# roljon/Steered-Mixture-of-Experts

Measured on AMD Instinct MI355X. Metric: Mpixel-iters/s (SMoE fit: forward + analytic backward + TF1 Adam), 16x16 blocks / 4 kernels, higher is better.
Workload: dtype f32

## Files before the change

### steered_mixture_of_experts_amd/csrc/smoe_block.hip.h

```cpp
#ifndef SMOE_BLOCK_HIP_H
#define SMOE_BLOCK_HIP_H

#include <hip/hip_runtime.h>
#include <stdint.h>

#include <type_traits>

#include "smoe_device.h"
#include "smoe_ssim.hip.h"
#include "smoe_fq.hip.h"

namespace smoe {


__device__ __forceinline__ float fast_rcp(float x) { return __builtin_amdgcn_rcpf(x); }

__device__ __forceinline__ uint32_t hw_wave_slot() {
    return __builtin_amdgcn_s_getreg(4 | (0 << 6) | ((4 - 1) << 11));
}
__device__ __forceinline__ void rotate_priority(int it, uint32_t slot) {
    const uint32_t pr = ((uint32_t)it + slot) % 3u;
    if (pr == 0u) __builtin_amdgcn_s_setprio(0);
    else if (pr == 1u) __builtin_amdgcn_s_setprio(1);
    else __builtin_amdgcn_s_setprio(2);
// ... 118 lines not shown
    __device__ __forceinline__ float nu(int k, int c) const { return P[k * Lt::PK + Lt::O_NU + c]; }
    __device__ __forceinline__ float ga(int k, int l, int c) const { return P[k * Lt::PK + Lt::O_GA + l * C + c]; }
    __device__ __forceinline__ bool flag(int k) const { return P[Lt::LP_ACT + k] != 0.0f; }
    __device__ __forceinline__ bool frozen() const { return P[Lt::LP_FROZEN] != 0.0f; }
    __device__ __forceinline__ bool act(int k) const { return flag(k) && (pi(k) > 0.0f); }

    __device__ __forceinline__ void load(const float* __restrict__ lds_block) {
        const float4* src = reinterpret_cast<const float4*>(lds_block);
#pragma unroll
        for (int i = 0; i < Lt::LP_STRIDE / 4; ++i) {
            const float4 q = src[i];
            P[4 * i + 0] = q.x; P[4 * i + 1] = q.y; P[4 * i + 2] = q.z; P[4 * i + 3] = q.w;
        }
    }

    template <bool IC = false>
    __device__ __forceinline__ void derive(const KernelConsts& kc) {
#pragma unroll
        for (int k = 0; k < K; ++k) {
            float det = 1.0f;
#pragma unroll
            for (int l = 0; l < D; ++l) det *= A(k, l, l);
            const float nq = kc.use_det ? det * kc.inv_n_dis : 1.0f;
            coef[k] = act(k) ? nq * pi(k) : 0.0f;
#pragma unroll
            for (int l = 0; l < D; ++l)
#pragma unroll
                for (int m = 0; m <= l; ++m)
                    As[k][tri_index(l, m)] = (IC ? ((l == m) ? SMOE_SQ * SMOE_SQ : 2.0f * SMOE_SQ * SMOE_SQ) : SMOE_SQ) * A(k, l, m);
#pragma unroll
            for (int m = 0; m < D; ++m) {
                float c = 0.0f;
                if (!IC) {
#pragma unroll
                    for (int l = m; l < D; ++l) c = fmaf(mu(k, l), As[k][tri_index(l, m)], c);
                }
                cz[k][m] = c;
            }
            if (!kc.train_gammas) {
#pragma unroll
                for (int i = 0; i < D * C; ++i) P[k * Lt::PK + Lt::O_GA + i] = 0.0f;
            }
            if (kc.only_y_gamma) {
#pragma unroll
// ... 156 lines not shown
            float h = R.nu(k, c);
#pragma unroll
            for (int l = D - HL; l < D; ++l) h = fmaf(R.ga(k, l, c), xc[l], h);
            R.he[k][c] = h;
        }
    }
}

template <int D, int C, int K>
struct PixelOut {
    float wt[K];
    float q[C];
    float kq[C];
};

template <int D, int C, int K, bool TRAIN, int HL = 0, bool EXTG = false, bool IC = false, bool FLAGS = false, bool RAWLOSS = false>
__device__ __forceinline__ void pixel(const BlockRegs<D, C, K>& R, const KernelConsts& kc,
                                      const float (&x)[D], const float (&t)[C], float lw,
                                      float* __restrict__ acc, PixelOut<D, C, K>& o,
                                      const float* __restrict__ gext = nullptr,
                                      unsigned long long* __restrict__ flags = nullptr, bool fed = true,
                                      float* __restrict__ lraw = nullptr, unsigned long long fedm = ~0ull) {
    using Lt = Layout<D, C, K>;
    float z[K][D], g[K];
    float S = 0.0f;
#pragma unroll
    for (int k = 0; k < K; ++k) {
        float maha = 0.0f;
        if (IC) {
            maha = (HL > 0) ? R.hq[k] : 0.0f;
#pragma unroll
// ... 37 lines not shown
#pragma unroll
            for (int l = 0; l < D - HL; ++l) ee = fmaf(R.ga(k, l, c), x[l], ee);
            e[k][c] = ee;
            y[c] = (k == 0) ? o.wt[k] * ee : fmaf(o.wt[k], ee, y[c]);
        }
    }
    float Gc[C];
    float dot = 0.0f;
#pragma unroll
    for (int c = 0; c < C; ++c) {
        const float yc = __builtin_amdgcn_fmed3f(y[c], 0.0f, kc.nudged_max);
        o.kq[c] = floorf(fmaf(yc, kc.inv_scale, 0.5f));
        o.q[c] = o.kq[c] * kc.scale;
        const float diff = o.q[c] - t[c];
        const float ad = fabsf(diff) - kc.epsm;
        acc[Lt::S_SSE] = fmaf(diff, diff, acc[Lt::S_SSE]);
        const float cwl = kc.cw[c] * lw;
        if constexpr (RAWLOSS) lraw[c] = fmaf(ad, ad, lraw[c]);
        else if (!EXTG) acc[Lt::S_LOSS] = fmaf(cwl, ad * ad, acc[Lt::S_LOSS]);
        if (TRAIN) {
            const float c2 = cwl + cwl;
            const float gm = EXTG ? gext[c] : ad * __builtin_amdgcn_fmed3f(diff * 1.2676506e30f, -c2, c2);
            Gc[c] = (yc == y[c]) ? gm : 0.0f;
            dot = (c == 0) ? Gc[c] * y[c] : fmaf(Gc[c], y[c], dot);
        }
    }
    if (!TRAIN) return;
    dot = (S > 10e-12f) ? dot : 0.0f;
    float Gx[(D - HL > 0) ? D - HL : 1][C];
#pragma unroll
    for (int l = 0; l < D - HL; ++l)
// ... 62 lines not shown
            for (int c = 0; c < C; ++c) a[Lt::O_GA + l * C + c] = xc[l] * a[Lt::O_NU + c];
        }
    }
}

template <int D, int C, int K>
__device__ __forceinline__ void tie_diagonal(float* __restrict__ a) {
    using Lt = Layout<D, C, K>;
    float tr = 0.0f;
#pragma unroll
    for (int l = 0; l < D; ++l) tr += a[Lt::O_A + tri_index(l, l)];
#pragma unroll
    for (int l = 0; l < D; ++l) a[Lt::O_A + tri_index(l, l)] = tr;
}

template <int D, int C, int K, bool IC = false>
__device__ __forceinline__ void finish_partials(const BlockRegs<D, C, K>& R, const KernelConsts& kc,
                                                float* __restrict__ acc) {
    using Lt = Layout<D, C, K>;
#pragma unroll
    for (int k = 0; k < K; ++k) {
        float* a = acc + k * Lt::PK;
        const bool act = R.act(k);
        const float su = a[Lt::O_PI];
        if (IC) {
            float sur[D];
#pragma unroll
            for (int l = 0; l < D; ++l) sur[l] = a[Lt::O_MU + l];
#pragma unroll
            for (int l = 0; l < D; ++l) {
                float gm = 0.0f;
#pragma unroll
                for (int m = 0; m < D; ++m) gm = fmaf((l >= m) ? R.A(k, l, m) : R.A(k, m, l), sur[m], gm);
                a[Lt::O_MU + l] = gm;
// ... 11 lines not shown
        float suz[D];
#pragma unroll
        for (int m = 0; m < D; ++m) suz[m] = a[Lt::O_MU + m] * SMOE_INV_SQ;
#pragma unroll
        for (int l = 0; l < D; ++l) {
            float gm = 0.0f;
#pragma unroll
            for (int m = 0; m <= l; ++m) gm = fmaf(R.A(k, l, m), suz[m], gm);
            a[Lt::O_MU + l] = gm;
        }
#pragma unroll
        for (int l = 0; l < D; ++l) {
#pragma unroll
            for (int m = 0; m <= l; ++m) {
                float v = fmaf(R.mu(k, l), suz[m], -(a[Lt::O_A + tri_index(l, m)] * SMOE_INV_SQ));
                if (l == m && kc.use_det) v = fmaf(su, act ? fast_rcp(R.A(k, l, l)) : 0.0f, v);
                a[Lt::O_A + tri_index(l, m)] = v;
            }
        }
        a[Lt::O_PI] = su * (act ? fast_rcp(R.pi(k)) : 0.0f);
        if (kc.radial) tie_diagonal<D, C, K>(a);
    }
}

struct SlotDesc {
    float c_self, pub_scale;
    uint32_t T1, T2, T3, TR, P1, P2, P3, PR, FLAG, PIV;
};

template <int D, int C, int K, bool IC>
__device__ __forceinline__ SlotDesc build_slot_desc(int j, uint32_t tot_base, uint32_t img_base, uint32_t par_base,
                                                    bool patch_pis, bool use_det) {
    using Lt = Layout<D, C, K>;
    const uint32_t ZERO = par_base + 4u * Lt::LP_ZERO, ONE = par_base + 4u * Lt::LP_ONE;
    const int k = j / Lt::PK, o = j - k * Lt::PK;
// ... 97 lines not shown
    __host__ __device__ static constexpr int tgt_stride(int N) { return C * N + TGT_PAD; }
    __host__ __device__ static constexpr int lw_stride(int N) { return N + TGT_PAD; }
    
    __host__ __device__ static int off_coords() { return 0; }
    __host__ __device__ static int off_par(int N, int CR) { return round_up(CR * N, 4); }
    __host__ __device__ static int off_mv(int N, int CR) { return off_par(N, CR) + NB * Lt::LP_STRIDE; }
    static constexpr bool OWNER_POST = (G >= 64);
    static constexpr int DESC_DW = 12;
    static constexpr int DESC_STRIDE = OWNER_POST ? Lt::NPAR * DESC_DW : 0;
    static constexpr int TOT_STRIDE = round_up(Lt::NSLOT, 4);
    static_assert(!OWNER_POST || BPW * TOT_STRIDE <= CH * ROW, "the published totals must fit into the reduction scratch");
    __host__ __device__ static bool wants_owner_post(int N) { return OWNER_POST && N <= 8 * G; }
    __host__ __device__ static int off_scratch(int N, int CR) { return off_mv(N, CR) + NB * MV_STRIDE; }
    __host__ __device__ static int off_tgt(int N, int CR) { return off_scratch(N, CR) + WAVES * CH * ROW; }
    __host__ __device__ static int off_lw(int N, int CR) { return off_tgt(N, CR) + NB * tgt_stride(N); }
    __host__ __device__ static size_t bytes(int N, bool has_lw, int CR = D, bool hq = false) {
        return sizeof(float) * (size_t)off_ssim(N, has_lw, CR, hq);
    }
    static constexpr int QI_RNG = 40;
    static constexpr int QI_OUT = 12;
    static constexpr int QI_STRIDE = round_up(Lt::LP_STRIDE + QI_RNG + QI_OUT, 4);
    __host__ __device__ static int off_qimg(int N, bool has_lw, int CR) { return round_up(off_lw(N, CR) + (has_lw ? NB * lw_stride(N) : 0), 4); }
    __host__ __device__ static int off_ssim(int N, bool has_lw, int CR, bool hq = false) { return off_qimg(N, has_lw, CR) + (hq ? NB * QI_STRIDE : 0); }
    __host__ __device__ static int ssim_tabs(int bh, int bw, int bt = 0) { return (G == 16) ? 0 : round_up(11 * (bh + bw + bt), 4); }
    __host__ __device__ static int ssim_wave(int N) { return (G == 16) ? BPW * C * N : round_up(C * N + ((D == 3) ? 10 : 8) * N, 4); }
    __host__ __device__ static size_t bytes_ssim(int N, bool has_lw, int CR, int bh, int bw, bool hq = false, int bt = 0) {
        return sizeof(float) * (size_t)(off_ssim(N, has_lw, CR, hq) + ssim_tabs(bh, bw, bt) + WAVES * ssim_wave(N));
    }
};

template <int D, int C, int K, int G, int WAVES, int CR = D>
__device__ __forceinline__ void stage_inputs(const float* __restrict__ coords, const float* __restrict__ target,
// ... 322 lines not shown
        float4 r = row[0];
#pragma unroll
        for (int i = 1; i < G / 4; ++i) {
            const float4 q = row[i];
            if (MIN) { r.x = fminf(r.x, q.x); r.y = fminf(r.y, q.y); r.z = fminf(r.z, q.z); r.w = fminf(r.w, q.w); }
            else { r.x += q.x; r.y += q.y; r.z += q.z; r.w += q.w; }
        }
        s_out[sub] = MIN ? fminf(fminf(r.x, r.y), fminf(r.z, r.w)) : (r.x + r.y) + (r.z + r.w);
    }
    wave_lds_sync();
#pragma unroll
    for (int i = 0; i < 10; ++i) v[i] = s_out[i];
    wave_lds_sync();
}

template <int D, int C, int K, bool HAS_LW, int HL, bool IC = false>
__device__ __forceinline__ void pixel_loop_train(const BlockRegs<D, C, K>& R, const KernelConsts& kc,
                                                 const float* __restrict__ s_coords, const float* __restrict__ s_tgt,
                                                 const float* __restrict__ s_lw, int N, int G, int sub,
                                                 float* __restrict__ acc, bool sample = false) {
    const int pxl = (N + G - 1) / G;
    const int full = N / G;
    unsigned long long flags[K];
#pragma unroll
    for (int k = 0; k < K; ++k) flags[k] = 0ull;
    constexpr bool RAWL = !HAS_LW;
    const unsigned long long not_sampled = sample ? 0ull : ~0ull;
    float lraw[C];
#pragma unroll
    for (int c = 0; c < C; ++c) lraw[c] = 0.0f;
    auto step = [&](int i) {
        const int n = i * G + sub;
        float x[D], t[C];
#pragma unroll
        for (int l = 0; l < D; ++l) x[l] = (l < D - HL) ? s_coords[l * N + n] : 0.0f;
#pragma unroll
        for (int c = 0; c < C; ++c) t[c] = s_tgt[c * N + n];
        const float lw = HAS_LW ? s_lw[n] : 1.0f;
        PixelOut<D, C, K> o;
        const bool fed = !(HAS_LW && sample) || lw != 0.0f;
        unsigned long long fedm = ~0ull;
        if constexpr (HAS_LW) fedm = __ballot(lw != 0.0f) | not_sampled;
        pixel<D, C, K, true, HL, false, IC, true, RAWL>(R, kc, x, t, lw, acc, o, nullptr, flags, fed, lraw, fedm);
    };
    int i = 0;
    if (full > 0) { step(0); i = 1; }
    if constexpr (D == 2 && C == 3) {
        for (; i < full; ++i) step(i);
    } else {
        for (; i + 1 < full; i += 2) { step(i); step(i + 1); }
        if (i < full) step(i);
    }
    if (full < pxl) {
        const int n = full * G + sub;
        if (n < N) {
            float x[D], t[C];
#pragma unroll
            for (int l = 0; l < D; ++l) x[l] = (l < D - HL) ? s_coords[l * N + n] : 0.0f;
#pragma unroll
            for (int c = 0; c < C; ++c) t[c] = s_tgt[c * N + n];
            const float lw = HAS_LW ? s_lw[n] : 1.0f;
            PixelOut<D, C, K> o;
            pixel<D, C, K, true, HL, false, IC, false, RAWL>(R, kc, x, t, lw, acc, o, nullptr, nullptr, !(HAS_LW && sample) || lw != 0.0f, lraw);
        }
    }
    if constexpr (RAWL) {
#pragma unroll
        for (int c = 0; c < C; ++c) acc[Layout<D, C, K>::S_LOSS] = fmaf(kc.cw[c], lraw[c], acc[Layout<D, C, K>::S_LOSS]);
    }
    const int lane = threadIdx.x & 63;
#pragma unroll
    for (int k = 0; k < K; ++k) acc[Layout<D, C, K>::S_CNT + k] += ((flags[k] >> lane) & 1ull) ? 1.0f : 0.0f;
}

template <int D, int C, int K, int G, int HL, bool SSIM, bool QUANT>
constexpr int fit_min_waves() {
    return ((G == 64 || (G == 16 && SMOE_W2_G16) || (G == 32 && SMOE_W2_G32)) && HL >= 1 && !SSIM && !QUANT && Layout<D, C, K>::NSLOT >= ((G == 64) ? SMOE_W2_SLOTS : 90)
            && Layout<D, C, K>::NSLOT <= SMOE_W2_SLOTS_MAX) ? 2 : 1;
}

template <int D, int C, int K, int G, int WAVES, int HL, bool SSIM = false, bool QUANT = false, bool IC = false, bool PAIR = false>
__global__ void __launch_bounds__(WAVES * 64) __attribute__((amdgpu_waves_per_eu(fit_min_waves<D, C, K, G, HL, SSIM, QUANT>()))) fit_kernel(FitArgs a) {
    using Lt = Layout<D, C, K>;
    using T = Tile<D, C, K, G, WAVES>;
    static_assert(!PAIR || (G == 64 && WAVES == 2 && !SSIM && !QUANT), "PAIR: one block on the two wavefronts of a workgroup");
    extern __shared__ __attribute__((aligned(16))) float lds[];
    const int N = a.N;
    const int B = a.B;
    const int wave = threadIdx.x >> 6;
    const int lane = threadIdx.x & 63;
    const int grp = lane / G;
    const int sub = lane - grp * G;
    const int blk0 = blockIdx.x * (PAIR ? 1 : T::NB);
    const int lb = PAIR ? 0 : wave * T::BPW + grp;
// ... 1 lines not shown
    const int b_raw = blk0 + lb;
    const bool valid_b = b_raw < B;
    const int b = valid_b ? b_raw : B - 1;

    constexpr int CR = D - HL;
    float* s_coords = lds + T::off_coords();
    float* s_par = lds + T::off_par(N, CR) + lb * Lt::LP_STRIDE;
    float* s_mv = lds + T::off_mv(N, CR) + lb * T::MV_STRIDE;
    float* s_scratch = lds + T::off_scratch(N, CR) + wave * (T::CH * T::ROW);
    const bool owner_post = T::OWNER_POST && a.desc_off > 0;
    float* s_desc = lds + a.desc_off + lb * T::DESC_STRIDE;
    float* s_tot = s_scratch + grp * T::TOT_STRIDE;
    const float* s_tgt = lds + T::off_tgt(N, CR) + lb * T::tgt_stride(N);
    const float* s_lw = lds + T::off_lw(N, CR) + lb * T::lw_stride(N);
    const bool has_lw = a.loss_w != nullptr;

    SMOE_LDS_CHECK(T::off_ssim(N, has_lw, CR, QUANT) + (SSIM ? T::ssim_tabs(a.bh, a.bw, (D == 3) ? a.bt : 0) + WAVES * T::ssim_wave(N) : 0), 1u);
    if (owner_post) SMOE_LDS_CHECK(a.desc_off + T::NB * T::DESC_STRIDE, 2u);
    stage_inputs<D, C, K, G, WAVES, CR>(a.coords, a.target, a.loss_w, B, N, blk0, lds);
    float* s_q = lds + T::off_qimg(N, has_lw, CR) + lb * T::QI_STRIDE;
    float* s_rng = s_q + Lt::LP_STRIDE;
    float* s_out = s_rng + T::QI_RNG;
    float* s_ssim = lds + T::off_ssim(N, has_lw, CR, QUANT);
    const int bh = a.bh, bw = a.bw, bt = (D == 3) ? a.bt : 0;
    const float* s_Tr = s_ssim;
    const float* s_Tc = s_ssim + bh * 11;
    const float* s_Tt = s_Tc + bw * 11;
    float* s_X = s_ssim + T::ssim_tabs(bh, bw, bt) + wave * T::ssim_wave(N) + ((G == 16) ? grp * (C * N) : 0);
    float* s_Wa = s_X + C * N;
    float* s_Wb = s_Wa + 5 * N;
    float wj[11];
    if (SSIM) {
// ... 30 lines not shown
            int tensor, kern; long off;
            decode_slot<D, C, K>(j, b, tensor, off, kern);
            s_par[j] = pick(a.p, tensor)[off];
            s_mv[2 * j] = pick(a.m, tensor)[off];
            s_mv[2 * j + 1] = pick(a.v, tensor)[off];
            float r = (tensor == 0) ? a.lr_pis : ((tensor == 2 || tensor == 3) ? a.lr_steer : a.lr_expert);
            if (tensor == 0 && !a.train_pis) r = 0.0f;
            if (tensor == 1 && !a.train_musx) r = 0.0f;
            if (tensor == 4 && !a.kc.train_gammas) r = 0.0f;
            if (tensor == 4 && a.kc.only_y_gamma && (off % C) != 0) r = 0.0f;
            if (tensor == 3 && a.kc.radial) r = 0.0f;
            lr[s] = r;
            reg[s] = (tensor == 0) ? a.reg_pi : ((tensor == 2) ? (a.kc.radial ? a.reg_u * (float)D : a.reg_u) : 0.0f);
            const int qg = (tensor == 0) ? 3 : ((tensor == 1) ? 1 : ((tensor == 4) ? 4 : ((tensor == 5) ? 2 : 0)));
            meta[s] = tensor | (kern << 4);
            if constexpr (QUANT) {
                if (tensor == 1 && a.mus_grid != nullptr && a.kc.qmode >= 2) goff[s] = a.mus_grid[off];
                if ((tensor == 0 && a.kc.qpis) || (tensor != 0 && a.kc.qmode == 2)) {
                    qlo[s] = a.kc.q_nmin[qg]; qhi[s] = a.kc.q_nmax[qg]; qsc[s] = a.kc.q_scale[qg]; qiv[s] = a.kc.q_inv[qg];
                }
                if (a.kc.qmode == 3 && tensor != 0 && !(tensor == 1 && !a.kc.q_musx))
                    qt[s] = (tensor == 2) ? 0 : ((tensor == 3) ? 1 : ((tensor == 1) ? 2 : ((tensor == 5) ? 3 : 4)));
            } else {
                (void)qg;
            }
        } else if (j >= Lt::S_CNT && j < Lt::S_CNT + K) {
            const int k = j - Lt::S_CNT;
            s_par[Lt::LP_ACT + k] = ((a.active[b] >> k) & 1u) ? 1.0f : 0.0f;
        } else if (j == Lt::S_LOSS) {
            s_par[Lt::LP_FROZEN] = (a.diverged != nullptr && a.diverged[b] != 0u) ? 1.0f : 0.0f;
        }
    }
    const float loss0 = (a.loss0 != nullptr) ? a.loss0[b] : 0.0f;
    const bool has_loss0 = a.loss0 != nullptr;
    const bool has_reg = (a.reg_pi != 0.0f) || (a.reg_u != 0.0f);
    const bool has_quant = (a.kc.qmode != 0) || (a.kc.qpis != 0);
    float last_loss = no_pass_value(), last_sse = no_pass_value();
    __syncthreads();

    auto pick5 = [](const float (&v)[10], int base, int t) {
        return (t == 0) ? v[base] : ((t == 1) ? v[base + 1] : ((t == 2) ? v[base + 2] : ((t == 3) ? v[base + 3] : v[base + 4])));
    };
    auto refresh_quantised_image = [&]() {
        if constexpr (QUANT) {
            if (a.kc.qmode == 3) {
                constexpr float INF = __builtin_huge_valf();
                float ex[10];
#pragma unroll
                for (int i = 0; i < 10; ++i) ex[i] = INF;
                const FqRange rp = fq_fixed(a.kc, 3);
#pragma unroll
                for (int s = 0; s < T::SPL; ++s) {
                    const int j = T::slot_of(sub, s);
                    if (j < Lt::NPAR && qt[s] >= 0) {
                        const bool keep = fq_val(s_par[(meta[s] >> 4) * Lt::PK + Lt::O_PI], rp) > 0.0f;
                        const float x = s_par[j] - goff[s];
#pragma unroll
                        for (int t = 0; t < 5; ++t) {
                            const bool hit = keep && (qt[s] == t);
                            ex[t] = hit ? fminf(ex[t], x) : ex[t];
                            ex[5 + t] = hit ? fminf(ex[5 + t], -x) : ex[5 + t];
                        }
                    }
                }
                block_allreduce10<G, T::ROW, true>(ex, s_scratch, s_out, lane, grp, sub);
                {
                    const int t = min(sub, 4);
                    float lo = pick5(ex, 0, t), hi = -pick5(ex, 5, t);
                    if (lo == INF) { lo = 0.0f; hi = 0.0f; }
                    if (t == 1) { lo = fminf(lo, 0.0f); hi = fmaxf(hi, 0.0f); }
// ... 3 lines not shown
                        float* o = s_rng + t * 8;
                        o[0] = r.nmin; o[1] = r.nmax; o[2] = r.scale; o[3] = r.inv;
                        o[4] = r.back; o[5] = r.zero ? 1.0f : 0.0f; o[6] = lo; o[7] = hi;
                    }
                }
                wave_lds_sync();
            }
        }
        if constexpr (!QUANT) {
#pragma unroll
            for (int s = 0; s < T::SPL; ++s) {
                const int j = T::slot_of(sub, s);
                if (meta[s] >= 0 && (meta[s] & 15) == 0) {
                    const float x = s_par[j];
                    const float cl = fminf(fmaxf(x, a.kc.q_nmin[3]), a.kc.q_nmax[3]);
                    s_par[Lt::LP_QPI + (meta[s] >> 4)] = floorf((cl - a.kc.q_nmin[3]) * a.kc.q_inv[3] + 0.5f) * a.kc.q_scale[3] + a.kc.q_nmin[3];
                }
            }
            wave_lds_sync();
            return;
        }
        if constexpr (QUANT) {
#pragma unroll
        for (int s = 0; s < T::SPL; ++s) {
            const int j = T::slot_of(sub, s);
            if (j < Lt::NPAR) {
                const float x = s_par[j] - goff[s];
                float q = x;
                if (qsc[s] != 0.0f) {
                    const float cl = fminf(fmaxf(x, qlo[s]), qhi[s]);
                    q = floorf((cl - qlo[s]) * qiv[s] + 0.5f) * qsc[s] + qlo[s];
// ... 8 lines not shown
                    }
                }
                s_q[j] = q + goff[s];
            } else if (j >= Lt::S_CNT && j < Lt::S_CNT + K) {
                s_q[Lt::LP_ACT + (j - Lt::S_CNT)] = s_par[Lt::LP_ACT + (j - Lt::S_CNT)];
            } else if (j == Lt::S_LOSS) {
                s_q[Lt::LP_FROZEN] = s_par[Lt::LP_FROZEN];
            }
        }
        }
        wave_lds_sync();
    };
    if (has_quant) refresh_quantised_image();
    const float* s_img = (QUANT && has_quant) ? s_q : s_par;
    const bool patch_pis = !QUANT && (a.kc.qpis != 0);
    if (owner_post && !helper) {
        const uint32_t tot_off = (uint32_t)((s_tot - lds) * sizeof(float));
        const uint32_t img_off = (uint32_t)((s_img - lds) * sizeof(float));
        const uint32_t par_off = (uint32_t)((s_par - lds) * sizeof(float));
#pragma unroll
        for (int s = 0; s < T::SPL; ++s) {
            const int j = T::slot_of(sub, s);
            if (j < Lt::NPAR) {
                const SlotDesc d = build_slot_desc<D, C, K, IC>(j, tot_off, img_off, par_off, patch_pis, a.kc.use_det != 0);
                float4* o = reinterpret_cast<float4*>(s_desc + j * T::DESC_DW);
                o[0] = make_float4(d.c_self, d.pub_scale, __uint_as_float(d.T1), __uint_as_float(d.T2));
                o[1] = make_float4(__uint_as_float(d.T3), __uint_as_float(d.TR), __uint_as_float(d.P1), __uint_as_float(d.P2));
                o[2] = make_float4(__uint_as_float(d.P3), __uint_as_float(d.PR), __uint_as_float(d.FLAG), __uint_as_float(d.PIV));
            } else if (j == Lt::S_LOSS) {
                s_par[Lt::LP_ZERO] = 0.0f;
// ... 16 lines not shown
    for (int it = 0; it < a.n_iters; ++it) {
        if (a.prio_rotate) rotate_priority(it, hw_wave_slot());
        else if (phase_prio) __builtin_amdgcn_s_setprio(0);
        float acc[Lt::NSLOT];
#pragma unroll
        for (int j = 0; j < Lt::NSLOT; ++j) acc[j] = 0.0f;
        bool frozen;
        float reg_loss = 0.0f;
        {
            BlockRegs<D, C, K> R;
            R.load(s_img);
            if (patch_pis) {
#pragma unroll
                for (int k = 0; k < K; ++k) R.P[k * Lt::PK + Lt::O_PI] = R.P[Lt::LP_QPI + k];
            }
            R.template derive<IC>(kc);
            frozen = R.frozen();
            if (has_reg) {
                const float rp = kc.kcount_norm ? kc.pis_l1_raw / count_pis<D, C, K>(R.P) : reg_pi;
#pragma unroll
                for (int k = 0; k < K; ++k) {
                    if (R.act(k)) {
                        reg_loss += rp * R.pi(k);
#pragma unroll
                        for (int l = 0; l < D; ++l) reg_loss += reg_u * R.A(k, l, l);
                    }
                }
            }
            if (HL > 0) hoist_const<D, C, K, HL, IC>(R, xc);
#if SMOE_SGPR_CONSTS
            if constexpr (G == 64 && !SSIM && !QUANT && !IC && HL >= 1 && K * C >= 24) {
// ... 42 lines not shown
                    float x[D], t[C], gq[C];
#pragma unroll
                    for (int l = 0; l < D; ++l) x[l] = (l < D - HL) ? s_coords[l * N + n] : 0.0f;
#pragma unroll
                    for (int c = 0; c < C; ++c) { t[c] = s_tgt[c * N + n]; gq[c] = s_X[c * N + n]; }
                    PixelOut<D, C, K> o;
                    pixel<D, C, K, true, HL, true, IC, decltype(voted)::value>(R, kc, x, t, 1.0f, acc, o, gq, flags);
                };
                for (int i = 0; i < full; ++i) grad_step(i * G + sub, std::true_type{});
                for (int i = full; i < pxl; ++i)
                    if (i * G + sub < N) grad_step(i * G + sub, std::false_type{});
#pragma unroll
                for (int k = 0; k < K; ++k) acc[Lt::S_CNT + k] += ((flags[k] >> lane) & 1ull) ? 1.0f : 0.0f;
            } else {
                const int gl = PAIR ? 2 * G : G, sl = PAIR ? wave * G + sub : sub;
                if (has_lw) pixel_loop_train<D, C, K, true, HL, IC>(R, kc, s_coords, s_tgt, s_lw, N, gl, sl, acc, a.lw_is_sample != 0);
                else pixel_loop_train<D, C, K, false, HL, IC>(R, kc, s_coords, s_tgt, s_lw, N, gl, sl, acc);
            }
            if (HL > 0) complete_const<D, C, K, HL, IC>(R, xc, acc);
            SMOE_CLK(1);
        }
        if (phase_prio) __builtin_amdgcn_s_setprio(3);
        if (!owner_post) {
            BlockRegs<D, C, K> R2;
            R2.load(s_img);
            if (patch_pis) {
#pragma unroll
                for (int k = 0; k < K; ++k) R2.P[k * Lt::PK + Lt::O_PI] = R2.P[Lt::LP_QPI + k];
            }
            finish_partials<D, C, K, IC>(R2, kc, acc);
        }

        SMOE_CLK(2);
        float total[T::SPL];
        reduce_slots<D, C, K, G, WAVES, 0>(acc, s_scratch, lane, total);
        SMOE_CLK(3);

        if constexpr (PAIR) {
            float* s_x = lds + T::off_scratch(N, CR) + (T::CH * T::ROW);
            if (helper) {
                wave_lds_sync();
#pragma unroll
                for (int s = 0; s < T::SPL; ++s) {
                    const int j = T::slot_of(sub, s);
                    if (j < Lt::NSLOT) s_x[j] = total[s];
// ... 90 lines not shown
            if (kc.qmode == 3) {
                float rs[10], cn[10];
                bool bel[T::SPL], abv[T::SPL], tlo[T::SPL], thi[T::SPL];
#pragma unroll
                for (int i = 0; i < 10; ++i) { rs[i] = 0.0f; cn[i] = 0.0f; }
                const FqRange rp = fq_fixed(kc, 3);
#pragma unroll
                for (int s = 0; s < T::SPL; ++s) {
                    const int j = T::slot_of(sub, s);
                    bel[s] = abv[s] = tlo[s] = thi[s] = false;
                    if (j < Lt::NPAR && qt[s] >= 0) {
                        const float* o = s_rng + qt[s] * 8;
                        const bool unshifted = qt[s] == 0 && kc.radial;
                        const float x = s_par[j] - goff[s], v = unshifted ? x : x - o[4];
                        const bool zero = o[5] != 0.0f;
                        const bool keep = fq_val(s_par[(meta[s] >> 4) * Lt::PK + Lt::O_PI], rp) > 0.0f;
                        bel[s] = !zero && (v < o[0]);
                        abv[s] = !zero && (v > o[1]);
                        tlo[s] = keep && (x == o[6]);
                        thi[s] = keep && (x == o[7]);
#pragma unroll
                        for (int t = 0; t < 5; ++t) {
                            const bool hit = qt[s] == t;
                            rs[t] += (hit && (unshifted ? !abv[s] : bel[s])) ? gq[s] : 0.0f;
                            rs[5 + t] += (hit && abv[s]) ? gq[s] : 0.0f;
                            cn[t] += (hit && tlo[s]) ? 1.0f : 0.0f;
                            cn[5 + t] += (hit && thi[s]) ? 1.0f : 0.0f;
                        }
                    }
                }
                block_allreduce10<G, T::ROW, false>(rs, s_scratch, s_out, lane, grp, sub);
// ... 30 lines not shown
                if (patch_pis && meta[s] >= 0 && (meta[s] & 15) == 0) gsum = (pv >= kc.q_nmin[3] && pv <= kc.q_nmax[3]) ? gsum : 0.0f;
            }
            if (clip > 0.0f) gsum = fminf(fmaxf(gsum, -clip), clip);
            const float alpha = lr[s] * bias;
            const float m2 = mv + (gsum - mv) * (1.0f - beta1);
            const float v2 = vv + (gsum * gsum - vv) * (1.0f - beta2);
            const float p2 = pv - (m2 * alpha) * fast_rcp(__builtin_amdgcn_sqrtf(v2) + adam_eps);
            const bool upd = (j < Lt::NPAR) && (lr[s] != 0.0f) && !frozen;
            newp[s] = upd ? p2 : pv;
            newm[s] = upd ? m2 : mv;
            newv[s] = upd ? v2 : vv;
            const float lossv = (SSIM ? 1.0f + total[s] : total[s]) + reg_loss;
            const bool is_loss = (j == Lt::S_LOSS) && !frozen;
            last_loss = is_loss ? lossv : last_loss;
            bad = bad || (is_loss && ((lossv != lossv) || (has_loss0 && (lossv + 1.0f > (loss0 + 100.0f) * 10.0f))));
            last_sse = ((j == Lt::S_SSE) && !frozen) ? total[s] : last_sse;
        }
        wave_lds_sync();
        SMOE_CLK(6);
#pragma unroll
        for (int s = 0; s < T::SPL; ++s) {
            const int j = T::slot_of(sub, s);
            if (j < Lt::NPAR) {
                s_par[j] = newp[s];
                s_mv[2 * j] = newm[s];
                s_mv[2 * j + 1] = newv[s];
                if constexpr (!QUANT) {
                    if (patch_pis && meta[s] >= 0 && (meta[s] & 15) == 0) {
                        const float cl = fminf(fmaxf(newp[s], kc.q_nmin[3]), kc.q_nmax[3]);
                        s_par[Lt::LP_QPI + (meta[s] >> 4)] = floorf((cl - kc.q_nmin[3]) * kc.q_inv[3] + 0.5f) * kc.q_scale[3] + kc.q_nmin[3];
                    }
                }
            } else if (j >= Lt::S_CNT && j < Lt::S_CNT + K) {
                if (!frozen) s_par[Lt::LP_ACT + (j - Lt::S_CNT)] = (total[s] > 0.0f) ? 1.0f : 0.0f;
            } else if (j == Lt::S_LOSS) {
                if (bad) s_par[Lt::LP_FROZEN] = 1.0f;
            }
        }
        wave_lds_sync();
        if constexpr (QUANT) {
            if (has_quant) refresh_quantised_image();
        }
        if constexpr (PAIR) __syncthreads();
        b1p *= beta1;
        b2p *= beta2;
        SMOE_CLK(7);
// ... 421 lines not shown
    int nb = 0;
    if (allow_lds(reinterpret_cast<const void*>(kern), lds) != hipSuccess) return -1;
    if (hipOccupancyMaxActiveBlocksPerMultiprocessor(&nb, kern, threads, lds) != hipSuccess) return -1;
    return nb;
}

template <typename Args>
struct Launch {
    void (*kern)(Args) = nullptr;
    int hl = 0;
    int threads = 0, nb = 1;
    size_t lds = 0;
    int desc_off = 0;
    int regt = 0;
};

template <int D, int C, int K, int G, int WAVES, bool SSIM, bool QUANT, bool IC, bool PAIR, int HMIN, int HMAX>
auto fit_kernel_at(int hl) -> void (*)(FitArgs) {
    if constexpr (HMAX > HMIN) {
        if (hl < HMAX) return fit_kernel_at<D, C, K, G, WAVES, SSIM, QUANT, IC, PAIR, HMIN, HMAX - 1>(hl);
    }
    return fit_kernel<D, C, K, G, WAVES, HMAX, SSIM, QUANT, IC, PAIR>;
}

template <int D, int C, int K, int G, int WAVES, bool SSIM, bool QUANT, bool IC, int OM, int HMAX>
auto forward_kernel_at(int hl) -> void (*)(FwdArgs) {
    if constexpr (HMAX > 0) {
        if (hl < HMAX) return forward_kernel_at<D, C, K, G, WAVES, SSIM, QUANT, IC, OM, HMAX - 1>(hl);
    }
    return forward_kernel<D, C, K, G, WAVES, SSIM, QUANT, IC, HMAX, OM>;
// ... 28 lines not shown
                              : fit_kernel_at<D, C, K, G, WAVES, false, true, false, false, 0, HMAX>(r.hl);
            } else {
                return r;
            }
        } else if (g.ic) {
            r.kern = fit_kernel_at<D, C, K, G, WAVES, false, false, true, false, 0, HMAX>(r.hl);
        } else {
            r.kern = fit_kernel_at<D, C, K, G, WAVES, false, false, false, false, 0, HMAX>(r.hl);
            if constexpr (G == 64 && WAVES == 2) {
                if (g.pair) {
                    r.kern = fit_kernel_at<D, C, K, G, WAVES, false, false, false, true, 0, HMAX>(r.hl);
                    r.nb = 1;
                }
            }
        }
        shm = T::bytes(N, has_lw, D - r.hl, g.quant);
    }
    if (T::wants_owner_post(N)) {
        r.desc_off = (int)(shm / sizeof(float));
        shm += sizeof(float) * (size_t)T::NB * T::DESC_STRIDE;
    }
    r.lds = shm;
    return r;
}

template <int D, int C, int K, int G, int WAVES, bool FULL>
Launch<FwdArgs> resolve_fwd(Graph g, int N, bool has_lw, int hoist, int bh, int bw, int bt) {
    using T = Tile<D, C, K, G, WAVES>;
    constexpr int HMAX = (D == 3) ? 2 : 1;
    Launch<FwdArgs> r;
    r.threads = T::THREADS;
// ... 35 lines not shown
    aa.desc_off = r.desc_off;
    return launch_with_lds(r.kern, (a.B + r.nb - 1) / r.nb, r.threads, r.lds, aa, st);
}

template <int D, int C, int K, int G, int WAVES, bool FULL>
hipError_t launch_fwd(const FwdArgs& a, Graph g, hipStream_t st) {
    const Launch<FwdArgs> r = resolve_fwd<D, C, K, G, WAVES, FULL>(g, a.N, a.loss_w != nullptr, a.hoist, a.bh, a.bw, a.bt);
    if (!r.kern) return hipErrorNotSupported;
    FwdArgs aa = a;
    aa.regt = r.regt;
    return launch_with_lds(r.kern, (a.B + r.nb - 1) / r.nb, r.threads, r.lds, aa, st);
}

template <int D, int C, int K, int G, int WAVES, bool FULL>
size_t lds_bytes(Graph g, int N, bool has_lw, int bh, int bw, int bt) {
    if (!g.ssim) return Tile<D, C, K, G, WAVES>::bytes(N, has_lw, D, g.quant);
    if (!FULL || !(D == 2 || (D == 3 && G == 64)) || (G == 16 && (bh != 16 || bw != 16))) return (size_t)-1;
    return Tile<D, C, K, G, WAVES>::bytes_ssim(N, has_lw, D, bh, bw, g.quant, (D == 3) ? bt : 0);
}

template <int D, int C, int K, int G, int WAVES, bool FULL>
int fit_occupancy(int N, bool has_lw, int hoist, bool pair) {
    Graph g = {};
    g.pair = pair;
    const Launch<FitArgs> r = resolve_fit<D, C, K, G, WAVES, FULL>(g, N, has_lw, hoist, 0, 0, 0);
    const int nb = resident_workgroups(r.kern, r.threads, r.lds);
    return (nb < 0) ? -1 : nb * WAVES;
}

#define SMOE_STR_(x) #x
#define SMOE_STR(x) SMOE_STR_(x)
// ... 11 lines not shown
```

Baseline: 410,000.

## Publish scaled A' and reciprocals to LDS at the Adam update, and skip SSE when unused

For the lean D=2/K=4 plain fit graph with G<64, the Adam update now writes SMOE_SQ*A and reciprocals of pi and the diagonal of A into a per-block LDS image. Per-lane derive and finish_partials read these values instead of recomputing them, which removes redundant rcp and multiply work repeated in every lane each iteration. The SSE accumulation is also compiled out when no sse_out is requested. This costs extra LDS per block, a trash cell for slots with no published value, and more bit-packing in meta[] along with its complexity.

```diff
diff --git a/steered_mixture_of_experts_amd/csrc/smoe_block.hip.h b/steered_mixture_of_experts_amd/csrc/smoe_block.hip.h
--- a/steered_mixture_of_experts_amd/csrc/smoe_block.hip.h
+++ b/steered_mixture_of_experts_amd/csrc/smoe_block.hip.h
@@ -156,8 +156,15 @@
         }
     }
 
-    template <bool IC = false>
-    __device__ __forceinline__ void derive(const KernelConsts& kc) {
+    template <bool IC = false, bool PUB = false>
+    __device__ __forceinline__ void derive(const KernelConsts& kc, const float* __restrict__ pub_as = nullptr) {
+        static_assert(!(IC && PUB), "the published image holds A' of the plain graph");
+        if constexpr (PUB) {
+#pragma unroll
+            for (int k = 0; k < K; ++k)
+#pragma unroll
+                for (int t = 0; t < Lt::TRI; ++t) As[k][t] = pub_as[k * Lt::TRI + t];
+        }
 #pragma unroll
         for (int k = 0; k < K; ++k) {
             float det = 1.0f;
@@ -165,11 +172,13 @@
             for (int l = 0; l < D; ++l) det *= A(k, l, l);
             const float nq = kc.use_det ? det * kc.inv_n_dis : 1.0f;
             coef[k] = act(k) ? nq * pi(k) : 0.0f;
+            if constexpr (!PUB) {
 #pragma unroll
             for (int l = 0; l < D; ++l)
 #pragma unroll
                 for (int m = 0; m <= l; ++m)
                     As[k][tri_index(l, m)] = (IC ? ((l == m) ? SMOE_SQ * SMOE_SQ : 2.0f * SMOE_SQ * SMOE_SQ) : SMOE_SQ) * A(k, l, m);
+            }
 #pragma unroll
             for (int m = 0; m < D; ++m) {
                 float c = 0.0f;
@@ -356,7 +365,7 @@
     float kq[C];
 };
 
-template <int D, int C, int K, bool TRAIN, int HL = 0, bool EXTG = false, bool IC = false, bool FLAGS = false, bool RAWLOSS = false>
+template <int D, int C, int K, bool TRAIN, int HL = 0, bool EXTG = false, bool IC = false, bool FLAGS = false, bool RAWLOSS = false, bool SSE = true>
 __device__ __forceinline__ void pixel(const BlockRegs<D, C, K>& R, const KernelConsts& kc,
                                       const float (&x)[D], const float (&t)[C], float lw,
                                       float* __restrict__ acc, PixelOut<D, C, K>& o,
@@ -424,7 +433,7 @@
         o.q[c] = o.kq[c] * kc.scale;
         const float diff = o.q[c] - t[c];
         const float ad = fabsf(diff) - kc.epsm;
-        acc[Lt::S_SSE] = fmaf(diff, diff, acc[Lt::S_SSE]);
+        if constexpr (SSE) acc[Lt::S_SSE] = fmaf(diff, diff, acc[Lt::S_SSE]);
         const float cwl = kc.cw[c] * lw;
         if constexpr (RAWLOSS) lraw[c] = fmaf(ad, ad, lraw[c]);
         else if (!EXTG) acc[Lt::S_LOSS] = fmaf(cwl, ad * ad, acc[Lt::S_LOSS]);
@@ -517,10 +526,11 @@
     for (int l = 0; l < D; ++l) a[Lt::O_A + tri_index(l, l)] = tr;
 }
 
-template <int D, int C, int K, bool IC = false>
+template <int D, int C, int K, bool IC = false, bool PUB = false>
 __device__ __forceinline__ void finish_partials(const BlockRegs<D, C, K>& R, const KernelConsts& kc,
-                                                float* __restrict__ acc) {
+                                                float* __restrict__ acc, const float* __restrict__ rc = nullptr) {
     using Lt = Layout<D, C, K>;
+    static_assert(!(IC && PUB), "the published image belongs to the plain graph");
 #pragma unroll
     for (int k = 0; k < K; ++k) {
         float* a = acc + k * Lt::PK;
@@ -562,11 +572,11 @@
 #pragma unroll
             for (int m = 0; m <= l; ++m) {
                 float v = fmaf(R.mu(k, l), suz[m], -(a[Lt::O_A + tri_index(l, m)] * SMOE_INV_SQ));
-                if (l == m && kc.use_det) v = fmaf(su, act ? fast_rcp(R.A(k, l, l)) : 0.0f, v);
+                if (l == m && kc.use_det) v = fmaf(su, act ? (PUB ? rc[k * (D + 1) + l] : fast_rcp(R.A(k, l, l))) : 0.0f, v);
                 a[Lt::O_A + tri_index(l, m)] = v;
             }
         }
-        a[Lt::O_PI] = su * (act ? fast_rcp(R.pi(k)) : 0.0f);
+        a[Lt::O_PI] = su * (act ? (PUB ? rc[k * (D + 1) + D] : fast_rcp(R.pi(k))) : 0.0f);
         if (kc.radial) tie_diagonal<D, C, K>(a);
     }
 }
@@ -694,8 +704,14 @@
     __host__ __device__ static int off_scratch(int N, int CR) { return off_mv(N, CR) + NB * MV_STRIDE; }
     __host__ __device__ static int off_tgt(int N, int CR) { return off_scratch(N, CR) + WAVES * CH * ROW; }
     __host__ __device__ static int off_lw(int N, int CR) { return off_tgt(N, CR) + NB * tgt_stride(N); }
-    __host__ __device__ static size_t bytes(int N, bool has_lw, int CR = D, bool hq = false) {
-        return sizeof(float) * (size_t)off_ssim(N, has_lw, CR, hq);
+    static constexpr bool PUBLISH = (G < 64);
+    static constexpr int PUB_R = K * Lt::TRI;
+    static constexpr int PUB_TRASH = PUB_R + K * (D + 1);
+    static constexpr int PUB_STRIDE = round_up(PUB_TRASH + 1, 4);
+    static_assert(4 * PUB_STRIDE < 2048, "the byte offsets of a slot's published cells are 12- and 11-bit fields of meta[]");
+    __host__ __device__ static int off_pub(int N, bool has_lw, int CR) { return off_qimg(N, has_lw, CR); }
+    __host__ __device__ static size_t bytes(int N, bool has_lw, int CR = D, bool hq = false, bool pub = false) {
+        return sizeof(float) * (size_t)(off_ssim(N, has_lw, CR, hq) + ((pub && PUBLISH) ? NB * PUB_STRIDE : 0));
     }
     static constexpr int QI_RNG = 40;
     static constexpr int QI_OUT = 12;
@@ -1048,7 +1064,7 @@
     wave_lds_sync();
 }
 
-template <int D, int C, int K, bool HAS_LW, int HL, bool IC = false>
+template <int D, int C, int K, bool HAS_LW, int HL, bool IC = false, bool SSE = true>
 __device__ __forceinline__ void pixel_loop_train(const BlockRegs<D, C, K>& R, const KernelConsts& kc,
                                                  const float* __restrict__ s_coords, const float* __restrict__ s_tgt,
                                                  const float* __restrict__ s_lw, int N, int G, int sub,
@@ -1075,7 +1091,7 @@
         const bool fed = !(HAS_LW && sample) || lw != 0.0f;
         unsigned long long fedm = ~0ull;
         if constexpr (HAS_LW) fedm = __ballot(lw != 0.0f) | not_sampled;
-        pixel<D, C, K, true, HL, false, IC, true, RAWL>(R, kc, x, t, lw, acc, o, nullptr, flags, fed, lraw, fedm);
+        pixel<D, C, K, true, HL, false, IC, true, RAWL, SSE>(R, kc, x, t, lw, acc, o, nullptr, flags, fed, lraw, fedm);
     };
     int i = 0;
     if (full > 0) { step(0); i = 1; }
@@ -1095,7 +1111,7 @@
             for (int c = 0; c < C; ++c) t[c] = s_tgt[c * N + n];
             const float lw = HAS_LW ? s_lw[n] : 1.0f;
             PixelOut<D, C, K> o;
-            pixel<D, C, K, true, HL, false, IC, false, RAWL>(R, kc, x, t, lw, acc, o, nullptr, nullptr, !(HAS_LW && sample) || lw != 0.0f, lraw);
+            pixel<D, C, K, true, HL, false, IC, false, RAWL, SSE>(R, kc, x, t, lw, acc, o, nullptr, nullptr, !(HAS_LW && sample) || lw != 0.0f, lraw);
         }
     }
     if constexpr (RAWL) {
@@ -1112,6 +1128,12 @@
     return ((G == 64 || (G == 16 && SMOE_W2_G16) || (G == 32 && SMOE_W2_G32)) && HL >= 1 && !SSIM && !QUANT && Layout<D, C, K>::NSLOT >= ((G == 64) ? SMOE_W2_SLOTS : 90)
             && Layout<D, C, K>::NSLOT <= SMOE_W2_SLOTS_MAX) ? 2 : 1;
 }
+
+template <bool PUB>
+__device__ __forceinline__ int meta_kern(int mt) { return PUB ? ((mt >> 4) & 15) : (mt >> 4); }
+
+template <int D, int C, int K, int HL>
+constexpr bool fit_lean() { return D == 2 && K == 4 && (HL >= 1 || C == 1); }
 
 template <int D, int C, int K, int G, int WAVES, int HL, bool SSIM = false, bool QUANT = false, bool IC = false, bool PAIR = false>
 __global__ void __launch_bounds__(WAVES * 64) __attribute__((amdgpu_waves_per_eu(fit_min_waves<D, C, K, G, HL, SSIM, QUANT>()))) fit_kernel(FitArgs a) {
@@ -1143,8 +1165,14 @@
     const float* s_tgt = lds + T::off_tgt(N, CR) + lb * T::tgt_stride(N);
     const float* s_lw = lds + T::off_lw(N, CR) + lb * T::lw_stride(N);
     const bool has_lw = a.loss_w != nullptr;
-
-    SMOE_LDS_CHECK(T::off_ssim(N, has_lw, CR, QUANT) + (SSIM ? T::ssim_tabs(a.bh, a.bw, (D == 3) ? a.bt : 0) + WAVES * T::ssim_wave(N) : 0), 1u);
+    constexpr bool DEF = !SSIM && !QUANT && !IC && !PAIR && fit_lean<D, C, K, HL>();
+    constexpr bool PUB = DEF && T::PUBLISH;
+    float* s_pub = lds + T::off_pub(N, has_lw, CR) + lb * T::PUB_STRIDE;
+    auto pub_a = [&](int mt) -> float& { return *reinterpret_cast<float*>(reinterpret_cast<char*>(s_pub) + ((mt >> 8) & 0xfff)); };
+    auto pub_r = [&](int mt) -> float& { return *reinterpret_cast<float*>(reinterpret_cast<char*>(s_pub) + (mt >> 20)); };
+
+    SMOE_LDS_CHECK(T::off_ssim(N, has_lw, CR, QUANT) + (PUB ? T::NB * T::PUB_STRIDE : 0)
+                   + (SSIM ? T::ssim_tabs(a.bh, a.bw, (D == 3) ? a.bt : 0) + WAVES * T::ssim_wave(N) : 0), 1u);
     if (owner_post) SMOE_LDS_CHECK(a.desc_off + T::NB * T::DESC_STRIDE, 2u);
     stage_inputs<D, C, K, G, WAVES, CR>(a.coords, a.target, a.loss_w, B, N, blk0, lds);
     float* s_q = lds + T::off_qimg(N, has_lw, CR) + lb * T::QI_STRIDE;
@@ -1205,6 +1233,13 @@
             reg[s] = (tensor == 0) ? a.reg_pi : ((tensor == 2) ? (a.kc.radial ? a.reg_u * (float)D : a.reg_u) : 0.0f);
             const int qg = (tensor == 0) ? 3 : ((tensor == 1) ? 1 : ((tensor == 4) ? 4 : ((tensor == 5) ? 2 : 0)));
             meta[s] = tensor | (kern << 4);
+            if constexpr (PUB) {
+                const int t = j - kern * Lt::PK - Lt::O_A;
+                const int l = (t >= 3) ? 2 : ((t >= 1) ? 1 : 0);
+                const int oa = (tensor == 2 || tensor == 3) ? kern * Lt::TRI + t : T::PUB_TRASH;
+                const int orc = (tensor == 0) ? T::PUB_R + kern * (D + 1) + D : ((tensor == 2) ? T::PUB_R + kern * (D + 1) + l : T::PUB_TRASH);
+                meta[s] |= ((4 * oa) << 8) | ((4 * orc) << 20);
+            }
             if constexpr (QUANT) {
                 if (tensor == 1 && a.mus_grid != nullptr && a.kc.qmode >= 2) goff[s] = a.mus_grid[off];
                 if ((tensor == 0 && a.kc.qpis) || (tensor != 0 && a.kc.qmode == 2)) {
@@ -1226,6 +1261,7 @@
     const bool has_loss0 = a.loss0 != nullptr;
     const bool has_reg = (a.reg_pi != 0.0f) || (a.reg_u != 0.0f);
     const bool has_quant = (a.kc.qmode != 0) || (a.kc.qpis != 0);
+    const bool want_sse = !DEF || a.sse_out != nullptr;
     float last_loss = no_pass_value(), last_sse = no_pass_value();
     __syncthreads();
 
@@ -1244,7 +1280,7 @@
                 for (int s = 0; s < T::SPL; ++s) {
                     const int j = T::slot_of(sub, s);
                     if (j < Lt::NPAR && qt[s] >= 0) {
-                        const bool keep = fq_val(s_par[(meta[s] >> 4) * Lt::PK + Lt::O_PI], rp) > 0.0f;
+                        const bool keep = fq_val(s_par[meta_kern<PUB>(meta[s]) * Lt::PK + Lt::O_PI], rp) > 0.0f;
                         const float x = s_par[j] - goff[s];
 #pragma unroll
                         for (int t = 0; t < 5; ++t) {
@@ -1278,7 +1314,7 @@
                 if (meta[s] >= 0 && (meta[s] & 15) == 0) {
                     const float x = s_par[j];
                     const float cl = fminf(fmaxf(x, a.kc.q_nmin[3]), a.kc.q_nmax[3]);
-                    s_par[Lt::LP_QPI + (meta[s] >> 4)] = floorf((cl - a.kc.q_nmin[3]) * a.kc.q_inv[3] + 0.5f) * a.kc.q_scale[3] + a.kc.q_nmin[3];
+                    s_par[Lt::LP_QPI + meta_kern<PUB>(meta[s])] = floorf((cl - a.kc.q_nmin[3]) * a.kc.q_inv[3] + 0.5f) * a.kc.q_scale[3] + a.kc.q_nmin[3];
                 }
             }
             wave_lds_sync();
@@ -1317,6 +1353,20 @@
     if (has_quant) refresh_quantised_image();
     const float* s_img = (QUANT && has_quant) ? s_q : s_par;
     const bool patch_pis = !QUANT && (a.kc.qpis != 0);
+    if constexpr (PUB) {
+#pragma unroll
+        for (int s = 0; s < T::SPL; ++s) {
+            const int j = T::slot_of(sub, s);
+            if (j < Lt::NPAR) {
+                const float pv = s_par[j];
+                const bool qpi = patch_pis && (meta[s] & 15) == 0;
+                const float rv = qpi ? s_par[Lt::LP_QPI + meta_kern<PUB>(meta[s])] : pv;
+                pub_a(meta[s]) = SMOE_SQ * pv;
+                pub_r(meta[s]) = fast_rcp(rv);
+            }
+        }
+        wave_lds_sync();
+    }
     if (owner_post && !helper) {
         const uint32_t tot_off = (uint32_t)((s_tot - lds) * sizeof(float));
         const uint32_t img_off = (uint32_t)((s_img - lds) * sizeof(float));
@@ -1363,7 +1413,7 @@
 #pragma unroll
                 for (int k = 0; k < K; ++k) R.P[k * Lt::PK + Lt::O_PI] = R.P[Lt::LP_QPI + k];
             }
-            R.template derive<IC>(kc);
+            R.template derive<IC, PUB>(kc, s_pub);
             frozen = R.frozen();
             if (has_reg) {
                 const float rp = kc.kcount_norm ? kc.pis_l1_raw / count_pis<D, C, K>(R.P) : reg_pi;
@@ -1436,8 +1486,13 @@
                 for (int k = 0; k < K; ++k) acc[Lt::S_CNT + k] += ((flags[k] >> lane) & 1ull) ? 1.0f : 0.0f;
             } else {
                 const int gl = PAIR ? 2 * G : G, sl = PAIR ? wave * G + sub : sub;
-                if (has_lw) pixel_loop_train<D, C, K, true, HL, IC>(R, kc, s_coords, s_tgt, s_lw, N, gl, sl, acc, a.lw_is_sample != 0);
-                else pixel_loop_train<D, C, K, false, HL, IC>(R, kc, s_coords, s_tgt, s_lw, N, gl, sl, acc);
+                if (DEF && !want_sse) {
+                    if (has_lw) pixel_loop_train<D, C, K, true, HL, IC, !DEF>(R, kc, s_coords, s_tgt, s_lw, N, gl, sl, acc, a.lw_is_sample != 0);
+                    else pixel_loop_train<D, C, K, false, HL, IC, !DEF>(R, kc, s_coords, s_tgt, s_lw, N, gl, sl, acc);
+                } else {
+                    if (has_lw) pixel_loop_train<D, C, K, true, HL, IC>(R, kc, s_coords, s_tgt, s_lw, N, gl, sl, acc, a.lw_is_sample != 0);
+                    else pixel_loop_train<D, C, K, false, HL, IC>(R, kc, s_coords, s_tgt, s_lw, N, gl, sl, acc);
+                }
             }
             if (HL > 0) complete_const<D, C, K, HL, IC>(R, xc, acc);
             SMOE_CLK(1);
@@ -1450,7 +1505,12 @@
 #pragma unroll
                 for (int k = 0; k < K; ++k) R2.P[k * Lt::PK + Lt::O_PI] = R2.P[Lt::LP_QPI + k];
             }
-            finish_partials<D, C, K, IC>(R2, kc, acc);
+            float rc[PUB ? K * (D + 1) : 1];
+            if constexpr (PUB) {
+#pragma unroll
+                for (int i = 0; i < K * (D + 1); ++i) rc[i] = s_pub[T::PUB_R + i];
+            }
+            finish_partials<D, C, K, IC, PUB>(R2, kc, acc, rc);
         }
 
         SMOE_CLK(2);
@@ -1571,7 +1631,7 @@
                         const bool unshifted = qt[s] == 0 && kc.radial;
                         const float x = s_par[j] - goff[s], v = unshifted ? x : x - o[4];
                         const bool zero = o[5] != 0.0f;
-                        const bool keep = fq_val(s_par[(meta[s] >> 4) * Lt::PK + Lt::O_PI], rp) > 0.0f;
+                        const bool keep = fq_val(s_par[meta_kern<PUB>(meta[s]) * Lt::PK + Lt::O_PI], rp) > 0.0f;
                         bel[s] = !zero && (v < o[0]);
                         abv[s] = !zero && (v > o[1]);
                         tlo[s] = keep && (x == o[6]);
@@ -1632,7 +1692,7 @@
             const bool is_loss = (j == Lt::S_LOSS) && !frozen;
             last_loss = is_loss ? lossv : last_loss;
             bad = bad || (is_loss && ((lossv != lossv) || (has_loss0 && (lossv + 1.0f > (loss0 + 100.0f) * 10.0f))));
-            last_sse = ((j == Lt::S_SSE) && !frozen) ? total[s] : last_sse;
+            last_sse = (want_sse && (j == Lt::S_SSE) && !frozen) ? total[s] : last_sse;
         }
         wave_lds_sync();
         SMOE_CLK(6);
@@ -1643,11 +1703,19 @@
                 s_par[j] = newp[s];
                 s_mv[2 * j] = newm[s];
                 s_mv[2 * j + 1] = newv[s];
+                float rv = newp[s];
                 if constexpr (!QUANT) {
                     if (patch_pis && meta[s] >= 0 && (meta[s] & 15) == 0) {
                         const float cl = fminf(fmaxf(newp[s], kc.q_nmin[3]), kc.q_nmax[3]);
-                        s_par[Lt::LP_QPI + (meta[s] >> 4)] = floorf((cl - kc.q_nmin[3]) * kc.q_inv[3] + 0.5f) * kc.q_scale[3] + kc.q_nmin[3];
+                        const float q = floorf((cl - kc.q_nmin[3]) * kc.q_inv[3] + 0.5f) * kc.q_scale[3] + kc.q_nmin[3];
+                        s_par[Lt::LP_QPI + meta_kern<PUB>(meta[s])] = q;
+                        if constexpr (PUB) rv = q;
                     }
+                }
+                (void)rv;
+                if constexpr (PUB) {
+                    pub_a(meta[s]) = SMOE_SQ * newp[s];
+                    pub_r(meta[s]) = fast_rcp(rv);
                 }
             } else if (j >= Lt::S_CNT && j < Lt::S_CNT + K) {
                 if (!frozen) s_par[Lt::LP_ACT + (j - Lt::S_CNT)] = (total[s] > 0.0f) ? 1.0f : 0.0f;
@@ -2099,6 +2167,9 @@
     int desc_off = 0;
     int regt = 0;
 };
+
+template <int D, int C, int K>
+constexpr bool fit_lean_at(int hl) { return (hl >= 2) ? fit_lean<D, C, K, 2>() : ((hl == 1) ? fit_lean<D, C, K, 1>() : fit_lean<D, C, K, 0>()); }
 
 template <int D, int C, int K, int G, int WAVES, bool SSIM, bool QUANT, bool IC, bool PAIR, int HMIN, int HMAX>
 auto fit_kernel_at(int hl) -> void (*)(FitArgs) {
@@ -2157,7 +2228,7 @@
                 }
             }
         }
-        shm = T::bytes(N, has_lw, D - r.hl, g.quant);
+        shm = T::bytes(N, has_lw, D - r.hl, g.quant, !g.quant && !g.ic && fit_lean_at<D, C, K>(r.hl));
     }
     if (T::wants_owner_post(N)) {
         r.desc_off = (int)(shm / sizeof(float));
@@ -2223,7 +2294,7 @@
 
 template <int D, int C, int K, int G, int WAVES, bool FULL>
 size_t lds_bytes(Graph g, int N, bool has_lw, int bh, int bw, int bt) {
-    if (!g.ssim) return Tile<D, C, K, G, WAVES>::bytes(N, has_lw, D, g.quant);
+    if (!g.ssim) return Tile<D, C, K, G, WAVES>::bytes(N, has_lw, D, g.quant, !g.quant && !g.ic && (fit_lean_at<D, C, K>(0) || fit_lean_at<D, C, K>(1) || fit_lean_at<D, C, K>(2)));
     if (!FULL || !(D == 2 || (D == 3 && G == 64)) || (G == 16 && (bh != 16 || bw != 16))) return (size_t)-1;
     return Tile<D, C, K, G, WAVES>::bytes_ssim(N, has_lw, D, bh, bw, g.quant, (D == 3) ? bt : 0);
 }
```

Measured after the change: 409,200. No clear change (-0.2%).
